# eloimoliner/BABE

Measured on AMD Instinct MI355X. Metric: audio-sec/s (blind BWE, 10 s @ 44.1 kHz clips, 35 EDM steps 2nd order), whole job, higher is better.
Workload: dtype f32

## Files before the change

### babe_amd/csrc/common.h

```cpp
#pragma once
#include <hip/hip_runtime.h>
#include <cstdio>
#include <cstring>
#include <cstdint>

#define BABE_OK 0
#define BABE_ERR_ARG -1
#define BABE_ERR_HIP -2
#define BABE_ERR_UNSUPPORTED -3

void babe_set_error(const char* fmt, ...);

#define BABE_CHECK_ARG(cond, ...)                      \
    do {                                               \
        if (!(cond)) {                                 \
            babe_set_error(__VA_ARGS__);               \
            return BABE_ERR_ARG;                       \
        }                                              \
    } while (0)

#define BABE_TRY(call)                                 \
    do {                                               \
        const int rc__ = (call);                       \
        if (rc__ != BABE_OK) return rc__;              \
    } while (0)

#define BABE_LAUNCH_CHECK()                                                       \
    do {                                                                          \
        hipError_t e__ = hipGetLastError();                                       \
        if (e__ != hipSuccess) {                                                  \
            babe_set_error("%s:%d HIP launch error: %s", __FILE__, __LINE__,      \
                           hipGetErrorString(e__));                               \
            return BABE_ERR_HIP;                                                  \
        }                                                                         \
    } while (0)

static inline int cdiv(long a, long b) { return (int)((a + b - 1) / b); }

#include <atomic>
#include <initializer_list>
static inline hipError_t babe_lds_optin(std::atomic<unsigned long long>& done, std::initializer_list<const void*> fns,
                                        int bytes) {
    int dev = 0;
    hipError_t e = hipGetDevice(&dev);
    if (e != hipSuccess) return e;
    const unsigned long long bit = 1ull << (dev & 63);
    if (done.load(std::memory_order_acquire) & bit) return hipSuccess;
    for (const void* f : fns) {
        e = hipFuncSetAttribute(f, hipFuncAttributeMaxDynamicSharedMemorySize, bytes);
        if (e != hipSuccess) return e;
    }
    done.fetch_or(bit, std::memory_order_release);
    return hipSuccess;
}

__device__ __forceinline__ long sgpr_pin(long v) {
    asm volatile("" : "+s"(v));
    return v;
}
struct ChanSrc {
    const float* p1;
    long d2, cs1, cs2;
    int split;
    __device__ __forceinline__ void init(const float* in, long bs, long cs, const float* in2, long bs2, long cs2_,
                                         int split_, int b) {
        p1 = in + (long)b * bs;
        d2 = sgpr_pin(in2 ? (long)((in2 + (long)b * bs2) - p1) : 0);
        cs1 = sgpr_pin(cs);
        cs2 = sgpr_pin(in2 ? cs2_ : cs);
        split = split_;
    }
    __device__ __forceinline__ const float* operator()(int ci) const {
        const bool first = ci < split;
        const long cs = first ? cs1 : cs2;
        const int c = first ? ci : ci - split;
        return p1 + ((first ? 0 : d2) + (long)c * cs);
    }
};

__device__ __forceinline__ double wave_sum(double v) {
#pragma unroll
    for (int o = 32; o > 0; o >>= 1) v += __shfl_xor(v, o, 64);
    return v;
}
__device__ __forceinline__ float wave_sumf(float v) {
#pragma unroll
    for (int o = 32; o > 0; o >>= 1) v += __shfl_xor(v, o, 64);
    return v;
}

template <int NW>
__device__ __forceinline__ double block_sum(double v, double* sh) {
    v = wave_sum(v);
    if ((threadIdx.x & 63) == 0) sh[threadIdx.x >> 6] = v;
    __syncthreads();
    double t = sh[0];
#pragma unroll
    for (int w = 1; w < NW; ++w) t += sh[w];
    return t;
}
```

### babe_amd/csrc/misc.hip

```cpp
#include "common.h"
#include "../../include/babe_hip.h"
#include "prof.h"
#include <cstdarg>
#include <vector>

static thread_local char g_err[512] = "";

void babe_set_error(const char* fmt, ...) {
    va_list ap;
    va_start(ap, fmt);
    vsnprintf(g_err, sizeof(g_err), fmt, ap);
    va_end(ap);
}
extern "C" const char* babe_last_error(void) { return g_err; }
extern "C" const char* babe_version(void) { return "babe_hip 0.1 (gfx950)"; }

namespace {
struct ProfRec { hipEvent_t e0, e1; int slot; void* stream; double flops; };
struct Prof {
    bool on = false;
    int conv_slot_override = -1;
    std::vector<ProfRec> rec;
    size_t used = 0;
    double bytes[BABE_NSLOTS] = {}, flops[BABE_NSLOTS] = {}, exec[BABE_NSLOTS] = {};
// ... 22 lines not shown
    r.stream = stream;
    r.flops = flops;
    (void)hipEventRecord(r.e0, (hipStream_t)stream);
    g_prof.bytes[slot] += bytes;
    g_prof.flops[slot] += flops;
    g_prof.exec[slot] += exec_flops;
    g_prof.open = true;
}
extern "C" void babe_prof_end(void* stream) {
    if (!g_prof.open) return;
    (void)hipEventRecord(g_prof.rec[g_prof.used++].e1, (hipStream_t)stream);
    g_prof.open = false;
}
extern "C" int babe_prof_nslots(void) { return BABE_NSLOTS; }
extern "C" const char* babe_prof_slot_name(int slot) { return (slot >= 0 && slot < BABE_NSLOTS) ? kSlotNames[slot] : ""; }
extern "C" int babe_prof_enable(int on) {
    if (on < 0) return g_prof.on ? 1 : 0;
    g_prof.on = on != 0;
    g_prof.open = false;
    return BABE_OK;
}
extern "C" int babe_prof_conv_slot(int slot) {
    g_prof.conv_slot_override = (slot >= 0 && slot < BABE_NSLOTS) ? slot : -1;
    return BABE_OK;
}
extern "C" int babe_prof_read(double* ms, double* bytes, double* flops, double* exec_flops, long* launches) {
    for (int i = 0; i < BABE_NSLOTS; ++i) {
        if (ms) ms[i] = 0;
        if (launches) launches[i] = 0;
    }
    for (size_t i = 0; i < g_prof.used; ++i) {
        ProfRec& r = g_prof.rec[i];
        if (hipEventSynchronize(r.e1) != hipSuccess) {
            babe_set_error("prof_read: hipEventSynchronize failed");
            return BABE_ERR_HIP;
        }
        float t = 0;
        (void)hipEventElapsedTime(&t, r.e0, r.e1);
        if (ms) ms[r.slot] += t;
        if (launches) launches[r.slot]++;
    }
    for (int i = 0; i < BABE_NSLOTS; ++i) {
        if (bytes) bytes[i] = g_prof.bytes[i];
        if (flops) flops[i] = g_prof.flops[i];
        if (exec_flops) exec_flops[i] = g_prof.exec[i];
        g_prof.bytes[i] = g_prof.flops[i] = g_prof.exec[i] = 0;
    }
    g_prof.used = 0;
    return BABE_OK;
}
extern "C" long babe_prof_timeline(double* t0_ms, double* t1_ms, int* slot, int* lane, double* flops, long cap) {
    std::vector<void*> streams;
    long n = 0;
    for (size_t i = 0; i < g_prof.used && n < cap; ++i, ++n) {
        ProfRec& r = g_prof.rec[i];
        if (hipEventSynchronize(r.e1) != hipSuccess) {
            babe_set_error("prof_timeline: hipEventSynchronize failed");
            return BABE_ERR_HIP;
        }
        float a = 0, b = 0;
        (void)hipEventElapsedTime(&a, g_prof.rec[0].e0, r.e0);
        (void)hipEventElapsedTime(&b, g_prof.rec[0].e0, r.e1);
        size_t k = 0;
        while (k < streams.size() && streams[k] != r.stream) ++k;
        if (k == streams.size()) streams.push_back(r.stream);
        if (t0_ms) t0_ms[n] = a;
        if (t1_ms) t1_ms[n] = b;
        if (slot) slot[n] = r.slot;
        if (lane) lane[n] = (int)k;
        if (flops) flops[n] = r.flops;
    }
    return n;
}
extern "C" long babe_prof_pending(void) { return (long)g_prof.used; }
extern "C" int babe_prof_dispatch_counts(long* counts, int reset) {
    for (int i = 0; i < BABE_NSLOTS; ++i) {
        if (counts) counts[i] = g_prof.dispatch[i];
        if (reset) g_prof.dispatch[i] = 0;
    }
    return BABE_OK;
}

namespace {
template <int V>
__global__ __launch_bounds__(256) void axpby4d_kernel(const float* __restrict__ in, long in_bs, long in_cs,
                                                      float* __restrict__ out, long out_bs, long out_cs, int C, long n,
                                                      float alpha, float beta) {
    const int b = blockIdx.y / C, c = blockIdx.y % C;
    const float* x = in + (long)b * in_bs + (long)c * in_cs;
    float* y = out + (long)b * out_bs + (long)c * out_cs;
    const long stride = (long)gridDim.x * blockDim.x * V;
    for (long i = ((long)blockIdx.x * blockDim.x + threadIdx.x) * V; i < n; i += stride) {
        if constexpr (V == 4) {
            typedef float f32x4 __attribute__((ext_vector_type(4)));
            f32x4 v = alpha * *reinterpret_cast<const f32x4*>(x + i);
            if (beta != 0.f) v += beta * *reinterpret_cast<const f32x4*>(y + i);
            *reinterpret_cast<f32x4*>(y + i) = v;
        } else {
            const float v = alpha * x[i];
            y[i] = (beta != 0.f) ? v + beta * y[i] : v;
        }
    }
}

__global__ __launch_bounds__(256) void axpby2_4d_kernel(const float* __restrict__ xin, long x_bs, long x_cs,
                                                        const float* __restrict__ yin, long y_bs, long y_cs,
                                                        float* __restrict__ out, long out_bs, long out_cs, int C, long n,
                                                        float alpha, float beta) {
    typedef float f32x4 __attribute__((ext_vector_type(4)));
    const int b = blockIdx.y / C, c = blockIdx.y % C;
    const float* x = xin + (long)b * x_bs + (long)c * x_cs;
    const float* y = yin + (long)b * y_bs + (long)c * y_cs;
    float* o = out + (long)b * out_bs + (long)c * out_cs;
    const long stride = (long)gridDim.x * blockDim.x * 4;
    for (long i = ((long)blockIdx.x * blockDim.x + threadIdx.x) * 4; i < n; i += stride) {
        const f32x4 xv = *reinterpret_cast<const f32x4*>(x + i), yv = *reinterpret_cast<const f32x4*>(y + i);
        f32x4 v;
#pragma unroll
        for (int e = 0; e < 4; ++e) {
#pragma clang fp contract(off)
            const float p = alpha * xv[e], q = beta * yv[e];
            v[e] = p + q;
        }
        *reinterpret_cast<f32x4*>(o + i) = v;
    }
}

__global__ __launch_bounds__(256) void fill4d_kernel(float* __restrict__ out, long out_bs, long out_cs, int C, long n, float value) {
    const int b = blockIdx.y / C, c = blockIdx.y % C;
    float* y = out + (long)b * out_bs + (long)c * out_cs;
    for (long i = (long)blockIdx.x * blockDim.x + threadIdx.x; i < n; i += (long)gridDim.x * blockDim.x) y[i] = value;
}

__global__ __launch_bounds__(256) void linear_kernel(const float* __restrict__ x, const float* __restrict__ W,
                                                     const float* __restrict__ bias, float* __restrict__ out, int B,
                                                     int K, int J, int relu) {
    const int j = blockIdx.x * 4 + (threadIdx.x >> 6);
    const int lane = threadIdx.x & 63;
    if (j >= J) return;
    for (int b = 0; b < B; ++b) {
        float s = 0.f;
        for (int k = lane; k < K; k += 64) s += x[(long)b * K + k] * W[(long)j * K + k];
        s = wave_sumf(s);
        if (lane == 0) {
            s += bias ? bias[j] : 0.f;
            if (relu) s = s > 0.f ? s : 0.f;
            out[(long)b * J + j] = s;
        }
    }
}

__global__ void rff_kernel(const float* __restrict__ cnoise, const float* __restrict__ freq, float* __restrict__ out,
                           int B, int R) {
    const int i = blockIdx.x * blockDim.x + threadIdx.x;
    if (i >= B * R) return;
    const int b = i / R, r = i % R;
    const float tab = (6.283185307179586f * cnoise[b]) * freq[r];
    out[(long)b * 2 * R + r] = sinf(tab);
    out[(long)b * 2 * R + R + r] = cosf(tab);
}
}

extern "C" int babe_axpby4d(const float* in, long in_bs, long in_cs, float* out, long out_bs, long out_cs, int B,
                            int C, int F, int T, float alpha, float beta, void* stream) {
    BABE_CHECK_ARG(in && out && B > 0 && C > 0 && F > 0 && T > 0, "axpby4d: bad arguments");
    BABE_CHECK_ARG((long)B * C <= 65535 && F <= 65535, "axpby4d: grid too large");
    const long n = (long)F * T;
    auto al16 = [](const void* p) { return ((uintptr_t)p & 15) == 0; };
    const bool v4 = (n % 4 == 0) && al16(in) && al16(out) && in_bs % 4 == 0 && in_cs % 4 == 0 && out_bs % 4 == 0 &&
                    out_cs % 4 == 0;
    BabeProfScope prof(BABE_SLOT_AXPBY, (beta != 0.f ? 12.0 : 8.0) * B * C * (double)n, 0, 0, stream);
    if (v4) {
        int bx = cdiv(n / 4, 256);
        if (bx > 64) bx = 64;
        hipLaunchKernelGGL(axpby4d_kernel<4>, dim3(bx, B * C), dim3(256), 0, (hipStream_t)stream, in, in_bs, in_cs, out,
                           out_bs, out_cs, C, n, alpha, beta);
    } else {
        int bx = cdiv(n, 256);
        if (bx > 64) bx = 64;
        hipLaunchKernelGGL(axpby4d_kernel<1>, dim3(bx, B * C), dim3(256), 0, (hipStream_t)stream, in, in_bs, in_cs, out,
                           out_bs, out_cs, C, n, alpha, beta);
    }
    BABE_LAUNCH_CHECK();
    return BABE_OK;
}

extern "C" int babe_axpby2_4d(const float* x, long x_bs, long x_cs, const float* y, long y_bs, long y_cs, float* out, long out_bs,
                              long out_cs, int B, int C, int F, int T, float alpha, float beta, void* stream) {
    BABE_CHECK_ARG(x && y && out && B > 0 && C > 0 && F > 0 && T > 0, "axpby2_4d: bad arguments");
    BABE_CHECK_ARG((long)B * C <= 65535, "axpby2_4d: grid too large");
    const long n = (long)F * T;
    auto al16 = [](const void* p) { return ((uintptr_t)p & 15) == 0; };
    BABE_CHECK_ARG(n % 4 == 0 && al16(x) && al16(y) && al16(out) && x_bs % 4 == 0 && x_cs % 4 == 0 && y_bs % 4 == 0 && y_cs % 4 == 0 &&
                       out_bs % 4 == 0 && out_cs % 4 == 0,
                   "axpby2_4d: planes must be 16-byte aligned with F*T %% 4 == 0 (use two babe_axpby4d calls otherwise)");
    BabeProfScope prof(BABE_SLOT_AXPBY, 12.0 * B * C * (double)n, 0, 0, stream);
    int bx = cdiv(n / 4, 256);
    if (bx > 64) bx = 64;
    hipLaunchKernelGGL(axpby2_4d_kernel, dim3(bx, B * C), dim3(256), 0, (hipStream_t)stream, x, x_bs, x_cs, y, y_bs, y_cs, out, out_bs,
                       out_cs, C, n, alpha, beta);
    BABE_LAUNCH_CHECK();
    return BABE_OK;
}

extern "C" int babe_fill4d(float* out, long out_bs, long out_cs, int B, int C, int F, int T, float value, void* stream) {
    BABE_CHECK_ARG(out && B > 0 && C > 0 && F > 0 && T > 0 && (long)B * C <= 65535, "fill4d: bad arguments");
    const long n = (long)F * T;
    int bx = cdiv(n, 1024);
    if (bx > 64) bx = 64;
    hipLaunchKernelGGL(fill4d_kernel, dim3(bx, B * C), dim3(256), 0, (hipStream_t)stream, out, out_bs, out_cs, C, n, value);
    BABE_LAUNCH_CHECK();
    return BABE_OK;
}

extern "C" int babe_linear(const float* x, const float* W, const float* bias, float* out, int B, int K, int J,
                           int relu, void* stream) {
    BABE_CHECK_ARG(x && W && out && B > 0 && K > 0 && J > 0, "linear: bad arguments");
    BabeProfScope prof(BABE_SLOT_FILM, 4.0 * ((double)J * K + (double)B * (K + J)), 2.0 * B * J * K, 0, stream);
    hipLaunchKernelGGL(linear_kernel, dim3(cdiv(J, 4)), dim3(256), 0, (hipStream_t)stream, x, W, bias, out, B, K, J,
                       relu);
    BABE_LAUNCH_CHECK();
    return BABE_OK;
}

extern "C" int babe_rff(const float* cnoise, const float* freq, float* out, int B, int R, void* stream) {
    BABE_CHECK_ARG(cnoise && freq && out && B > 0 && R > 0, "rff: bad arguments");
    BabeProfScope prof(BABE_SLOT_FILM, 4.0 * B * (1 + 3 * R), 0, 0, stream);
    hipLaunchKernelGGL(rff_kernel, dim3(cdiv(B * R, 64)), dim3(64), 0, (hipStream_t)stream, cnoise, freq, out, B, R);
    BABE_LAUNCH_CHECK();
    return BABE_OK;
}
```

### babe_amd/csrc/norm.hip

```cpp
#include "common.h"
#include "../../include/babe_hip.h"
#include "prof.h"
#include "gelu.h"
#include <cstdlib>

namespace {

using babe_gelu::gelu_f;
using babe_gelu::gelu_grad_f;

template <int NV>
__device__ __forceinline__ void block_reduce(double (&v)[NV], double* sh) {
#pragma unroll
    for (int k = 0; k < NV; ++k) v[k] = wave_sum(v[k]);
    const int lane = threadIdx.x & 63, wave = threadIdx.x >> 6;
    if (lane == 0) {
#pragma unroll
        for (int k = 0; k < NV; ++k) sh[wave * NV + k] = v[k];
    }
    __syncthreads();
    if (threadIdx.x == 0) {
#pragma unroll
        for (int k = 0; k < NV; ++k) v[k] = 0;
        for (int w = 0; w < (int)(blockDim.x >> 6); ++w) {
#pragma unroll
            for (int k = 0; k < NV; ++k) v[k] += sh[w * NV + k];
        }
    }
}

struct GnStat {
    float mean, sd, r;
};
__device__ __forceinline__ GnStat gn_stat(double s0, double s1, long n, float eps) {
    const double mean = s0 / (double)n;
    double var = (s1 - (double)n * mean * mean) / (double)(n - 1);
    if (var < 0) var = 0;
    const float sd = (float)sqrt(var);
    return {(float)mean, sd, 1.f / (sd + eps)};
}
__device__ __forceinline__ void gn_stat_store(float* __restrict__ stats, int bg, const GnStat st) {
    stats[bg * 3 + 0] = st.mean;
    stats[bg * 3 + 1] = st.sd;
    stats[bg * 3 + 2] = st.r;
}

__device__ __forceinline__ void half_wave_sum2(double& s0, double& s1) {
#pragma unroll
    for (int o = 16; o >= 1; o >>= 1) {
        s0 += __shfl_xor(s0, o, 32);
        s1 += __shfl_xor(s1, o, 32);
    }
}
template <typename P>
__device__ __forceinline__ void gn_part_sum32(P part, long row, int S, int sub, double& s0, double& s1) {
    s0 = 0, s1 = 0;
    for (int q = sub; q < S; q += 32) {
        s0 += part[(row + q) * 2];
        s1 += part[(row + q) * 2 + 1];
    }
    half_wave_sum2(s0, s1);
}

template <bool FUSED>
__global__ __launch_bounds__(256) void gn_partial_kernel(const float* __restrict__ x, double* __restrict__ part,
                                                         long n, int S, int* __restrict__ ticket,
                                                         const float* __restrict__ gamma, const float* __restrict__ film,
                                                         long film_bs, float* __restrict__ stats, float* __restrict__ scale,
                                                         int C, int G, float eps) {
    __shared__ double sh[8];
    __shared__ int last_sh;
    __shared__ float r_sh;
    const int s = blockIdx.x;
    const long bg = blockIdx.y;
    const long chunk = ((n / 4 + S - 1) / S) * 4;
    const long beg = (long)s * chunk;
    long end = beg + chunk;
    if (end > n) end = n;
    const float* p = x + bg * n;
    double s0 = 0, s1 = 0;
    if (beg < end) {
        const long nv = (end - beg) / 4;
        const float4* p4 = reinterpret_cast<const float4*>(p + beg);
        long i = threadIdx.x;
        for (; i + 3 * (long)blockDim.x < nv; i += 4 * (long)blockDim.x) {
            const float4 v0 = p4[i], v1 = p4[i + blockDim.x], v2 = p4[i + 2 * blockDim.x], v3 = p4[i + 3 * blockDim.x];
            s0 += ((double)v0.x + (double)v0.y + (double)v0.z + (double)v0.w) + ((double)v1.x + (double)v1.y + (double)v1.z + (double)v1.w) +
                  ((double)v2.x + (double)v2.y + (double)v2.z + (double)v2.w) + ((double)v3.x + (double)v3.y + (double)v3.z + (double)v3.w);
            s1 += ((double)v0.x * v0.x + (double)v0.y * v0.y + (double)v0.z * v0.z + (double)v0.w * v0.w) +
                  ((double)v1.x * v1.x + (double)v1.y * v1.y + (double)v1.z * v1.z + (double)v1.w * v1.w) +
                  ((double)v2.x * v2.x + (double)v2.y * v2.y + (double)v2.z * v2.z + (double)v2.w * v2.w) +
                  ((double)v3.x * v3.x + (double)v3.y * v3.y + (double)v3.z * v3.z + (double)v3.w * v3.w);
        }
        for (; i < nv; i += blockDim.x) {
            const float4 v = p4[i];
            s0 += (double)v.x + (double)v.y + (double)v.z + (double)v.w;
            s1 += (double)v.x * v.x + (double)v.y * v.y + (double)v.z * v.z + (double)v.w * v.w;
        }
        for (long i = beg + nv * 4 + threadIdx.x; i < end; i += blockDim.x) {
            const double v = p[i];
            s0 += v;
            s1 += v * v;
        }
    }
    double sum[2] = {s0, s1};
    block_reduce(sum, sh);
    if (threadIdx.x == 0) {
        part[(bg * S + s) * 2] = sum[0];
        part[(bg * S + s) * 2 + 1] = sum[1];
    }
    if constexpr (FUSED) {
        if (threadIdx.x == 0) {
            __threadfence();
            const int old = atomicAdd(&ticket[bg], 1);
            last_sh = old == S - 1;
            if (old == S - 1) ticket[bg] = 0;
        }
        __syncthreads();
        if (!last_sh) return;
        __threadfence();
        const int b = (int)(bg / G), g = (int)(bg % G);
        if (threadIdx.x < 32) {
            const volatile double* vp = part;
            double t0, t1;
            gn_part_sum32(vp, bg * S, S, threadIdx.x, t0, t1);
            if (threadIdx.x == 0) {
                const GnStat st = gn_stat(t0, t1, n, eps);
                gn_stat_store(stats, b * G + g, st);
                r_sh = st.r;
            }
        }
        __syncthreads();
        const int cg = C / G;
        for (int j = threadIdx.x; j < cg; j += blockDim.x) {
            const int c = g * cg + j;
            scale[b * C + c] = gamma[c] * (film[(long)b * film_bs + c] + 1.f) * r_sh;
        }
    }
}

__global__ void gn_finalize_kernel(const double* __restrict__ part, const float* __restrict__ gamma,
                                   const float* __restrict__ film, long film_bs, float* __restrict__ stats,
                                   float* __restrict__ scale, int C, int G, long n, int S, float eps) {
    const int b = blockIdx.x;
    __shared__ float rstd_sh[64];
    const int sub = threadIdx.x & 31;
    for (int g = threadIdx.x >> 5; g < G; g += blockDim.x >> 5) {
        double s0, s1;
        gn_part_sum32(part, (long)(b * G + g) * S, S, sub, s0, s1);
        if (sub != 0) continue;
        const GnStat st = gn_stat(s0, s1, n, eps);
        gn_stat_store(stats, b * G + g, st);
        rstd_sh[g] = st.r;
    }
    __syncthreads();
    const int cg = C / G;
    for (int c = threadIdx.x; c < C; c += blockDim.x)
        scale[b * C + c] = gamma[c] * (film[(long)b * film_bs + c] + 1.f) * rstd_sh[c / cg];
}

__global__ __launch_bounds__(256) void scale_gelu_kernel(const float* __restrict__ x, const float* __restrict__ scale,
                                                         float* __restrict__ a, int C, long hw) {
    const int c = blockIdx.y, b = blockIdx.z;
    const float sc = scale[b * C + c];
    const long base = ((long)b * C + c) * hw;
    const long nv = hw / 4;
    const float4* x4 = reinterpret_cast<const float4*>(x + base);
    float4* a4 = reinterpret_cast<float4*>(a + base);
    for (long i = (long)blockIdx.x * blockDim.x + threadIdx.x; i < nv; i += (long)gridDim.x * blockDim.x) {
        float4 v = x4[i];
        v.x = gelu_f(v.x * sc);
        v.y = gelu_f(v.y * sc);
        v.z = gelu_f(v.z * sc);
        v.w = gelu_f(v.w * sc);
        a4[i] = v;
    }
    if (blockIdx.x == 0)
        for (long i = nv * 4 + threadIdx.x; i < hw; i += blockDim.x) a[base + i] = gelu_f(x[base + i] * sc);
}

__global__ __launch_bounds__(256) void scale_gelu_fin_kernel(const float* __restrict__ x, const double* __restrict__ part,
                                                             const float* __restrict__ gamma, const float* __restrict__ film,
                                                             long film_bs, float* __restrict__ stats, float* __restrict__ scale,
                                                             float* __restrict__ a, int C, int G, long hw, long n, int S,
                                                             float eps) {
    __shared__ float sc_sh;
    __shared__ double red_sh[512];
    const int c = blockIdx.y, b = blockIdx.z;
    const int cg = C / G, g = c / cg;
    {
        double t0 = 0, t1 = 0;
        for (int q = threadIdx.x; q < S; q += 256) {
            t0 += part[((long)(b * G + g) * S + q) * 2];
            t1 += part[((long)(b * G + g) * S + q) * 2 + 1];
        }
        red_sh[threadIdx.x * 2] = t0;
        red_sh[threadIdx.x * 2 + 1] = t1;
    }
    __syncthreads();
    if (threadIdx.x < 32) {
        double t0 = 0, t1 = 0;
#pragma unroll
        for (int j = 0; j < 8; ++j) {
            t0 += red_sh[(threadIdx.x + 32 * j) * 2];
            t1 += red_sh[(threadIdx.x + 32 * j) * 2 + 1];
        }
        half_wave_sum2(t0, t1);
        if (threadIdx.x == 0) {
            const GnStat st = gn_stat(t0, t1, n, eps);
            const float scv = gamma[c] * (film[(long)b * film_bs + c] + 1.f) * st.r;
            sc_sh = scv;
            if (blockIdx.x == 0) {
                scale[b * C + c] = scv;
                if (c == g * cg) gn_stat_store(stats, b * G + g, st);
            }
        }
    }
    __syncthreads();
    const float sc = sc_sh;
    const long base = ((long)b * C + c) * hw;
    const long nv = hw / 4;
    const float4* x4 = reinterpret_cast<const float4*>(x + base);
    float4* a4 = reinterpret_cast<float4*>(a + base);
    for (long i = (long)blockIdx.x * blockDim.x + threadIdx.x; i < nv; i += (long)gridDim.x * blockDim.x) {
        float4 v = x4[i];
        v.x = gelu_f(v.x * sc);
        v.y = gelu_f(v.y * sc);
        v.z = gelu_f(v.z * sc);
        v.w = gelu_f(v.w * sc);
        a4[i] = v;
    }
    if (blockIdx.x == 0)
        for (long i = nv * 4 + threadIdx.x; i < hw; i += blockDim.x) a[base + i] = gelu_f(x[base + i] * sc);
}

typedef __bf16 bf16x8_n __attribute__((ext_vector_type(8)));
__global__ __launch_bounds__(256) void scale_gelu_units_kernel(const float* __restrict__ x, const float* __restrict__ scale,
                                                               bf16x8_n* __restrict__ au, int C, int F, int T) {
    const int g = blockIdx.y, b = blockIdx.z;
    const int Q = T >> 2, PI = Q + 1;
    const long hw = (long)F * T;
    float sc[8];
#pragma unroll
    for (int j = 0; j < 8; ++j) sc[j] = scale[b * C + 8 * g + j];
    const float* xb = x + ((long)b * C + 8 * g) * hw;
    bf16x8_n* ab = au + ((long)b * (C >> 3) + g) * F * 4 * PI;
    const long nq = (long)F * Q;
    for (long i = (long)blockIdx.x * blockDim.x + threadIdx.x; i < nq; i += (long)gridDim.x * blockDim.x) {
        const int f = (int)(i / Q), q = (int)(i - (long)f * Q);
        float4 v[8];
#pragma unroll
        for (int j = 0; j < 8; ++j) v[j] = *reinterpret_cast<const float4*>(xb + j * hw + (long)f * T + 4 * q);
        bf16x8_n u0, u1, u2, u3, z;
#pragma unroll
        for (int j = 0; j < 8; ++j) {
            u0[j] = (__bf16)gelu_f(v[j].x * sc[j]);
            u1[j] = (__bf16)gelu_f(v[j].y * sc[j]);
            u2[j] = (__bf16)gelu_f(v[j].z * sc[j]);
            u3[j] = (__bf16)gelu_f(v[j].w * sc[j]);
            z[j] = (__bf16)0.f;
        }
        bf16x8_n* row = ab + (long)f * 4 * PI;
        row[1 * PI + q] = u0;
        row[2 * PI + q] = u1;
        row[3 * PI + q] = u2;
        row[q + 1] = u3;
        if (q == 0) row[0] = z;
        if (q == Q - 1) {
            row[1 * PI + Q] = z;
            row[2 * PI + Q] = z;
            row[3 * PI + Q] = z;
        }
    }
}

template <bool GELU>
__global__ __launch_bounds__(256) void gn_bwd_partial_kernel(const float* __restrict__ x, const float* __restrict__ dadu,
                                                             const float* __restrict__ scale,
                                                             double* __restrict__ part, int C, int G, long hw, int S) {
    __shared__ double sh[4];
    const int s = blockIdx.x;
    const int bg = blockIdx.y;
    const int b = bg / G, g = bg % G;
    const int cg = C / G;
    const long n = (long)cg * hw;
    const long chunk = ((n / 4 + S - 1) / S) * 4;
    const long beg = (long)s * chunk;
    long end = beg + chunk;
    if (end > n) end = n;
    const long base = ((long)b * C + (long)g * cg) * hw;
    double s0 = 0;
    if (beg < end) {
        const int c_lo = (int)(beg / hw), c_hi = (int)((end - 1) / hw);
        for (int cl = c_lo; cl <= c_hi; ++cl) {
            const long lo = beg > (long)cl * hw ? beg : (long)cl * hw;
            const long hi = end < (long)(cl + 1) * hw ? end : (long)(cl + 1) * hw;
            const float sc = scale[b * C + g * cg + cl];
            double sc_sum = 0;
            auto term = [&](const float4 xv, float4 dv) {
                if (GELU) {
                    dv.x *= gelu_grad_f(xv.x * sc);
                    dv.y *= gelu_grad_f(xv.y * sc);
                    dv.z *= gelu_grad_f(xv.z * sc);
                    dv.w *= gelu_grad_f(xv.w * sc);
                }
                return (double)dv.x * xv.x + (double)dv.y * xv.y + (double)dv.z * xv.z + (double)dv.w * xv.w;
            };
            const long st = (long)blockDim.x * 4;
            long i = lo + (long)threadIdx.x * 4;
            for (; i + st < hi; i += 2 * st) {
                const float4 x0 = *reinterpret_cast<const float4*>(x + base + i);
                const float4 d0 = *reinterpret_cast<const float4*>(dadu + base + i);
                const float4 x1 = *reinterpret_cast<const float4*>(x + base + i + st);
                const float4 d1 = *reinterpret_cast<const float4*>(dadu + base + i + st);
                sc_sum += term(x0, d0);
                sc_sum += term(x1, d1);
            }
            for (; i < hi; i += st)
                sc_sum += term(*reinterpret_cast<const float4*>(x + base + i), *reinterpret_cast<const float4*>(dadu + base + i));
            s0 += (double)sc * sc_sum;
        }
    }
    double sum[1] = {s0};
    block_reduce(sum, sh);
    if (threadIdx.x == 0) part[(long)bg * S + s] = sum[0];
}

template <bool GELU>
__global__ __launch_bounds__(256) void gn_bwd_apply_kernel(const float* __restrict__ x, const float* __restrict__ da,
                                                           const float* __restrict__ gy,
                                                           const float* __restrict__ scale,
                                                           const float* __restrict__ stats,
                                                           const double* __restrict__ part, float* __restrict__ gx,
                                                           float rbeta, int C, int G, long hw, int S, float eps,
                                                           const float* __restrict__ acc, float ca, float cb) {
    const int c = blockIdx.y, b = blockIdx.z;
    const int cg = C / G;
    const int g = c / cg;
    const long n = (long)cg * hw;
    __shared__ double S1_sh;
    if (threadIdx.x < 64) {
        double v = 0;
        for (int s = threadIdx.x; s < S; s += 64) v += part[(long)(b * G + g) * S + s];
        v = wave_sum(v);
        if (threadIdx.x == 0) S1_sh = v;
    }
    __syncthreads();
    const double S1 = S1_sh;
    const float mean = stats[(b * G + g) * 3 + 0];
    const float sd = stats[(b * G + g) * 3 + 1];
    const double se = (double)sd + eps;
    const float coef = (sd > 0.f) ? (float)(S1 * se / ((double)(n - 1) * sd * se * se)) : 0.f;
    const float sc = scale[b * C + c];
    const long base = ((long)b * C + c) * hw;
    const long nv = hw / 4;
    const float4* x4 = reinterpret_cast<const float4*>(x + base);
    const float4* d4 = reinterpret_cast<const float4*>(da + base);
    const float4* g4 = gy ? reinterpret_cast<const float4*>(gy + base) : nullptr;
    float4* o4 = reinterpret_cast<float4*>(gx + base);
    for (long i = (long)blockIdx.x * blockDim.x + threadIdx.x; i < nv; i += (long)gridDim.x * blockDim.x) {
        const float4 xv = x4[i];
        float4 dv = d4[i];
        if (GELU) {
            dv.x *= gelu_grad_f(xv.x * sc);
            dv.y *= gelu_grad_f(xv.y * sc);
            dv.z *= gelu_grad_f(xv.z * sc);
            dv.w *= gelu_grad_f(xv.w * sc);
        }
        float4 o;
        o.x = sc * dv.x - (xv.x - mean) * coef;
        o.y = sc * dv.y - (xv.y - mean) * coef;
        o.z = sc * dv.z - (xv.z - mean) * coef;
        o.w = sc * dv.w - (xv.w - mean) * coef;
        if (g4) {
            const float4 gv = g4[i];
            o.x += rbeta * gv.x;
            o.y += rbeta * gv.y;
            o.z += rbeta * gv.z;
            o.w += rbeta * gv.w;
        }
        if (acc) {
#pragma clang fp contract(off)
            const float4 av = reinterpret_cast<const float4*>(acc + base)[i];
            const float px = ca * av.x, py = ca * av.y, pz = ca * av.z, pw = ca * av.w;
            const float qx = cb * o.x, qy = cb * o.y, qz = cb * o.z, qw = cb * o.w;
            o.x = px + qx;
            o.y = py + qy;
            o.z = pz + qz;
            o.w = pw + qw;
        }
        o4[i] = o;
    }
}

int plane_blocks(long hw) {
    const int bx = cdiv(hw / 4, 256 * 4);
    return bx < 1 ? 1 : bx > 64 ? 64 : bx;
}

}

extern "C" long babe_gn_splits(long n) {
    const long s = n / 16384;
    return s < 1 ? 1 : s > 64 ? 64 : s;
}

extern "C" int babe_gn_partial(const float* x, double* part, int B, int G, long n, int S, void* stream) {
    BABE_CHECK_ARG(x && part && B > 0 && G > 0 && n > 1 && S > 0, "gn_partial: bad arguments");
    BABE_CHECK_ARG(n % 4 == 0, "gn_partial: group size %ld not a multiple of 4", n);
    BabeProfScope prof(BABE_SLOT_GN_STATS, 4.0 * B * G * (double)n, 0, 0, stream);
    hipLaunchKernelGGL(gn_partial_kernel<false>, dim3(S, B * G), dim3(256), 0, (hipStream_t)stream, x, part, n, S,
                       (int*)nullptr, (const float*)nullptr, (const float*)nullptr, 0L, (float*)nullptr, (float*)nullptr, 0, 1, 0.f);
    BABE_LAUNCH_CHECK();
    return BABE_OK;
}

extern "C" int babe_gn_stats(const float* x, double* part, int* ticket, const float* gamma, const float* film, long film_bs,
                             float* stats, float* scale, int B, int C, int G, long n, int S, float eps, void* stream) {
    BABE_CHECK_ARG(x && part && ticket && gamma && film && stats && scale && B > 0 && G > 0 && n > 1 && S > 0, "gn_stats: bad arguments");
    BABE_CHECK_ARG(n % 4 == 0 && G <= 64 && C % G == 0, "gn_stats: n=%ld C=%d G=%d unsupported", n, C, G);
    BabeProfScope prof(BABE_SLOT_GN_STATS, 4.0 * B * G * (double)n, 0, 0, stream);
    hipLaunchKernelGGL(gn_partial_kernel<true>, dim3(S, B * G), dim3(256), 0, (hipStream_t)stream, x, part, n, S, ticket, gamma,
                       film, film_bs, stats, scale, C, G, eps);
    BABE_LAUNCH_CHECK();
    return BABE_OK;
}

extern "C" int babe_gn_finalize(const double* part, const float* gamma, const float* film, long film_bs, float* stats,
                                float* scale, int B, int C, int G, long n, int S, float eps, void* stream) {
    BABE_CHECK_ARG(part && gamma && film && stats && scale, "gn_finalize: null pointer");
    BABE_CHECK_ARG(G <= 64 && C % G == 0, "gn_finalize: C=%d G=%d unsupported", C, G);
    BabeProfScope prof(BABE_SLOT_GN_STATS, 0, 0, 0, stream);
    hipLaunchKernelGGL(gn_finalize_kernel, dim3(B), dim3(256), 0, (hipStream_t)stream, part, gamma, film, film_bs,
                       stats, scale, C, G, n, S, eps);
    BABE_LAUNCH_CHECK();
    return BABE_OK;
}

extern "C" int babe_scale_gelu(const float* x, const float* scale, float* a, int B, int C, long hw, void* stream) {
    BABE_CHECK_ARG(x && scale && a && B > 0 && C > 0 && hw > 0, "scale_gelu: bad arguments");
    BABE_CHECK_ARG(hw % 4 == 0, "scale_gelu: plane size %ld not a multiple of 4", hw);
    BabeProfScope prof(BABE_SLOT_SCALE_GELU, 8.0 * B * C * (double)hw, 0, 0, stream);
    const int bx = plane_blocks(hw);
    hipLaunchKernelGGL(scale_gelu_kernel, dim3(bx, C, B), dim3(256), 0, (hipStream_t)stream, x, scale, a, C, hw);
    BABE_LAUNCH_CHECK();
    return BABE_OK;
}

extern "C" int babe_scale_gelu_fin(const float* x, const double* part, const float* gamma, const float* film, long film_bs,
                                   float* stats, float* scale, float* a, int B, int C, int G, long hw, int S, float eps,
                                   void* stream) {
    BABE_CHECK_ARG(x && part && gamma && film && stats && scale && a && B > 0 && C > 0 && hw > 0 && S > 0, "scale_gelu_fin: bad arguments");
    BABE_CHECK_ARG(hw % 4 == 0 && G <= 64 && C % G == 0, "scale_gelu_fin: hw=%ld C=%d G=%d unsupported", hw, C, G);
    BabeProfScope prof(BABE_SLOT_SCALE_GELU, 8.0 * B * C * (double)hw, 0, 0, stream);
    const int bx = plane_blocks(hw);
    const long n = (long)(C / G) * hw;
    hipLaunchKernelGGL(scale_gelu_fin_kernel, dim3(bx, C, B), dim3(256), 0, (hipStream_t)stream, x, part, gamma, film, film_bs,
                       stats, scale, a, C, G, hw, n, S, eps);
    BABE_LAUNCH_CHECK();
    return BABE_OK;
}

extern "C" long babe_units_size(int C, int F, int T) { return (long)(C / 8) * F * 4 * (T / 4 + 1); }

extern "C" int babe_scale_gelu_units(const float* x, const float* scale, void* au, int B, int C, int F, int T,
                                     void* stream) {
    BABE_CHECK_ARG(x && scale && au && B > 0 && C > 0 && F > 0 && T > 0, "scale_gelu_units: bad arguments");
    BABE_CHECK_ARG(T % 4 == 0 && C % 8 == 0, "scale_gelu_units: T=%d C=%d unsupported (need T %% 4 == 0, C %% 8 == 0)", T, C);
    BABE_CHECK_ARG(((uintptr_t)x & 15) == 0 && ((uintptr_t)au & 15) == 0, "scale_gelu_units: unaligned pointer");
    BabeProfScope prof(BABE_SLOT_SCALE_GELU, 6.0 * B * C * (double)F * T, 0, 0, stream);
    int bx = cdiv((long)F * (T / 4), 256 * 2);
    if (bx < 1) bx = 1;
    if (bx > 256) bx = 256;
    hipLaunchKernelGGL(scale_gelu_units_kernel, dim3(bx, C / 8, B), dim3(256), 0, (hipStream_t)stream, x, scale,
                       (bf16x8_n*)au, C, F, T);
    BABE_LAUNCH_CHECK();
    return BABE_OK;
}

static int gn_bwd_partial_launch(bool gelu, const float* x, const float* da, const float* scale, double* part, int B, int C, int G,
                                 long hw, int S, void* stream) {
    BABE_CHECK_ARG(x && da && scale && part, "gn_bwd_partial: null pointer");
    BABE_CHECK_ARG(hw % 4 == 0 && C % G == 0, "gn_bwd_partial: hw=%ld C=%d G=%d unsupported", hw, C, G);
    BabeProfScope prof(BABE_SLOT_GN_BWD_PARTIAL, 8.0 * B * C * (double)hw, 0, 0, stream);
    if (gelu)
        hipLaunchKernelGGL(gn_bwd_partial_kernel<true>, dim3(S, B * G), dim3(256), 0, (hipStream_t)stream, x, da, scale, part, C, G,
                           hw, S);
    else
        hipLaunchKernelGGL(gn_bwd_partial_kernel<false>, dim3(S, B * G), dim3(256), 0, (hipStream_t)stream, x, da, scale, part, C, G,
                           hw, S);
    BABE_LAUNCH_CHECK();
    return BABE_OK;
}

extern "C" int babe_gn_bwd_partial(const float* x, const float* da, const float* scale, double* part, int B, int C,
                                   int G, long hw, int S, void* stream) {
    return gn_bwd_partial_launch(true, x, da, scale, part, B, C, G, hw, S, stream);
}

extern "C" int babe_gn_bwd_partial_nogelu(const float* x, const float* da, const float* scale, double* part, int B, int C,
                                          int G, long hw, int S, void* stream) {
    return gn_bwd_partial_launch(false, x, da, scale, part, B, C, G, hw, S, stream);
}

static int gn_bwd_apply_launch(bool gelu, const float* acc, float ca, float cb, const float* x, const float* da, const float* gy, const float* scale,
                                 const float* stats, const double* part, float* gx, float rbeta, int B, int C, int G,
                                 long hw, int S, float eps, void* stream) {
    BABE_CHECK_ARG(x && da && scale && stats && part && gx, "gn_bwd_apply: null pointer");
    BABE_CHECK_ARG(hw % 4 == 0 && C % G == 0, "gn_bwd_apply: hw=%ld C=%d G=%d unsupported", hw, C, G);
    BabeProfScope prof(BABE_SLOT_GN_BWD_APPLY, ((gy ? 16.0 : 12.0) + (acc ? 4.0 : 0.0)) * B * C * (double)hw, 0, 0, stream);
    const int bx = plane_blocks(hw);
    if (gelu)
        hipLaunchKernelGGL(gn_bwd_apply_kernel<true>, dim3(bx, C, B), dim3(256), 0, (hipStream_t)stream, x, da, gy, scale, stats,
                           part, gx, rbeta, C, G, hw, S, eps, acc, ca, cb);
    else
        hipLaunchKernelGGL(gn_bwd_apply_kernel<false>, dim3(bx, C, B), dim3(256), 0, (hipStream_t)stream, x, da, gy, scale, stats,
                           part, gx, rbeta, C, G, hw, S, eps, acc, ca, cb);
    BABE_LAUNCH_CHECK();
    return BABE_OK;
}

extern "C" int babe_gn_bwd_apply(const float* x, const float* da, const float* gy, const float* scale,
                                 const float* stats, const double* part, float* gx, float rbeta, int B, int C, int G,
                                 long hw, int S, float eps, void* stream) {
    return gn_bwd_apply_launch(true, nullptr, 0.f, 0.f, x, da, gy, scale, stats, part, gx, rbeta, B, C, G, hw, S, eps, stream);
}

extern "C" int babe_gn_bwd_apply_nogelu(const float* x, const float* da, const float* gy, const float* scale,
                                        const float* stats, const double* part, float* gx, float rbeta, int B, int C, int G,
                                        long hw, int S, float eps, void* stream) {
    return gn_bwd_apply_launch(false, nullptr, 0.f, 0.f, x, da, gy, scale, stats, part, gx, rbeta, B, C, G, hw, S, eps, stream);
}

extern "C" int babe_gn_bwd_apply_merge(const float* x, const float* da, const float* gy, const float* scale,
                                 const float* stats, const double* part, float* gx, float rbeta, int B, int C, int G,
                                 long hw, int S, float eps, void* stream, const float* acc, float ca, float cb) {
    BABE_CHECK_ARG(acc && ((uintptr_t)acc & 15) == 0, "gn_bwd_apply_merge: acc must be a 16-byte aligned dense tensor");
    return gn_bwd_apply_launch(true, acc, ca, cb, x, da, gy, scale, stats, part, gx, rbeta, B, C, G, hw, S, eps, stream);
}
```

Before: 2.595.

## Software-pipeline elementwise and groupnorm kernels with double-buffered prefetch loads

```diff
diff --git a/babe_amd/csrc/common.h b/babe_amd/csrc/common.h
--- a/babe_amd/csrc/common.h
+++ b/babe_amd/csrc/common.h
@@ -89,6 +89,37 @@
     return v;
 }
 
+__device__ __forceinline__ void pipeline_head() {
+    asm volatile("" ::: "memory");
+    __builtin_amdgcn_sched_barrier(0);
+}
+
+__device__ __forceinline__ float4 ld16(const float* base, int i) {
+    return *reinterpret_cast<const float4*>(reinterpret_cast<const char*>(base) + (unsigned)i * 16u);
+}
+__device__ __forceinline__ void st16(float* base, int i, const float4 v) {
+    *reinterpret_cast<float4*>(reinterpret_cast<char*>(base) + (unsigned)i * 16u) = v;
+}
+
+template <typename T, typename Load, typename Use>
+__device__ __forceinline__ void sweep2(T a, T b, int i, const int st, const int nv, Load load, Use use) {
+    for (; i + 3 * st < nv; i += 2 * st) {
+        use(a, i);
+        a = load(i + 2 * st);
+        pipeline_head();
+        use(b, i + st);
+        b = load(i + 3 * st);
+        pipeline_head();
+    }
+    if (i < nv) {
+        use(a, i);
+        const bool third = i + 2 * st < nv;
+        if (third) a = load(i + 2 * st);
+        if (i + st < nv) use(b, i + st);
+        if (third) use(a, i + 2 * st);
+    }
+}
+
 template <int NW>
 __device__ __forceinline__ double block_sum(double v, double* sh) {
     v = wave_sum(v);
diff --git a/babe_amd/csrc/misc.hip b/babe_amd/csrc/misc.hip
--- a/babe_amd/csrc/misc.hip
+++ b/babe_amd/csrc/misc.hip
@@ -128,24 +128,53 @@
 }
 
 namespace {
-template <int V>
+typedef float f32x4 __attribute__((ext_vector_type(4)));
+__device__ __forceinline__ f32x4 ld16v(const float* base, int i) {
+    return *reinterpret_cast<const f32x4*>(reinterpret_cast<const char*>(base) + (unsigned)i * 16u);
+}
+__device__ __forceinline__ void st16v(float* base, int i, const f32x4 v) {
+    *reinterpret_cast<f32x4*>(reinterpret_cast<char*>(base) + (unsigned)i * 16u) = v;
+}
+
+template <bool BETA>
+__device__ __forceinline__ float axpby_one(float alpha, float x, float beta, float y) {
+    float p;
+    {
+#pragma clang fp contract(off)
+        p = alpha * x;
+    }
+    return BETA ? __builtin_fmaf(beta, y, p) : p;
+}
+
+template <int V, bool BETA>
 __global__ __launch_bounds__(256) void axpby4d_kernel(const float* __restrict__ in, long in_bs, long in_cs,
                                                       float* __restrict__ out, long out_bs, long out_cs, int C, long n,
                                                       float alpha, float beta) {
     const int b = blockIdx.y / C, c = blockIdx.y % C;
     const float* x = in + (long)b * in_bs + (long)c * in_cs;
     float* y = out + (long)b * out_bs + (long)c * out_cs;
-    const long stride = (long)gridDim.x * blockDim.x * V;
-    for (long i = ((long)blockIdx.x * blockDim.x + threadIdx.x) * V; i < n; i += stride) {
-        if constexpr (V == 4) {
-            typedef float f32x4 __attribute__((ext_vector_type(4)));
-            f32x4 v = alpha * *reinterpret_cast<const f32x4*>(x + i);
-            if (beta != 0.f) v += beta * *reinterpret_cast<const f32x4*>(y + i);
-            *reinterpret_cast<f32x4*>(y + i) = v;
-        } else {
-            const float v = alpha * x[i];
-            y[i] = (beta != 0.f) ? v + beta * y[i] : v;
-        }
+    if constexpr (V == 4) {
+        struct In {
+            f32x4 x, y;
+        };
+        const int nv = (int)(n / 4), i0 = blockIdx.x * blockDim.x + threadIdx.x, st = gridDim.x * blockDim.x;
+        auto load = [&](int i) {
+            In v;
+            v.x = ld16v(x, i);
+            if constexpr (BETA) v.y = ld16v(y, i);
+            return v;
+        };
+        const In in0 = load(i0 < nv ? i0 : nv - 1), in1 = load(i0 + st < nv ? i0 + st : nv - 1);
+        sweep2(in0, in1, i0, st, nv, load, [&](const In& in, int i) {
+            f32x4 v;
+#pragma unroll
+            for (int e = 0; e < 4; ++e) v[e] = axpby_one<BETA>(alpha, in.x[e], beta, BETA ? in.y[e] : 0.f);
+            st16v(y, i, v);
+        });
+    } else {
+        const long stride = (long)gridDim.x * blockDim.x;
+        for (long i = (long)blockIdx.x * blockDim.x + threadIdx.x; i < n; i += stride)
+            y[i] = axpby_one<BETA>(alpha, x[i], beta, BETA ? y[i] : 0.f);
     }
 }
 
@@ -153,23 +182,26 @@
                                                         const float* __restrict__ yin, long y_bs, long y_cs,
                                                         float* __restrict__ out, long out_bs, long out_cs, int C, long n,
                                                         float alpha, float beta) {
-    typedef float f32x4 __attribute__((ext_vector_type(4)));
     const int b = blockIdx.y / C, c = blockIdx.y % C;
     const float* x = xin + (long)b * x_bs + (long)c * x_cs;
     const float* y = yin + (long)b * y_bs + (long)c * y_cs;
     float* o = out + (long)b * out_bs + (long)c * out_cs;
-    const long stride = (long)gridDim.x * blockDim.x * 4;
-    for (long i = ((long)blockIdx.x * blockDim.x + threadIdx.x) * 4; i < n; i += stride) {
-        const f32x4 xv = *reinterpret_cast<const f32x4*>(x + i), yv = *reinterpret_cast<const f32x4*>(y + i);
+    struct In {
+        f32x4 x, y;
+    };
+    const int nv = (int)(n / 4), i0 = blockIdx.x * blockDim.x + threadIdx.x, st = gridDim.x * blockDim.x;
+    auto load = [&](int i) { return In{ld16v(x, i), ld16v(y, i)}; };
+    const In in0 = load(i0 < nv ? i0 : nv - 1), in1 = load(i0 + st < nv ? i0 + st : nv - 1);
+    sweep2(in0, in1, i0, st, nv, load, [&](const In& in, int i) {
         f32x4 v;
 #pragma unroll
         for (int e = 0; e < 4; ++e) {
 #pragma clang fp contract(off)
-            const float p = alpha * xv[e], q = beta * yv[e];
+            const float p = alpha * in.x[e], q = beta * in.y[e];
             v[e] = p + q;
         }
-        *reinterpret_cast<f32x4*>(o + i) = v;
-    }
+        st16v(o, i, v);
+    });
 }
 
 __global__ __launch_bounds__(256) void fill4d_kernel(float* __restrict__ out, long out_bs, long out_cs, int C, long n, float value) {
@@ -212,6 +244,7 @@
     BABE_CHECK_ARG(in && out && B > 0 && C > 0 && F > 0 && T > 0, "axpby4d: bad arguments");
     BABE_CHECK_ARG((long)B * C <= 65535 && F <= 65535, "axpby4d: grid too large");
     const long n = (long)F * T;
+    BABE_CHECK_ARG(n < (1L << 30), "axpby4d: plane of %ld elements too large", n);
     auto al16 = [](const void* p) { return ((uintptr_t)p & 15) == 0; };
     const bool v4 = (n % 4 == 0) && al16(in) && al16(out) && in_bs % 4 == 0 && in_cs % 4 == 0 && out_bs % 4 == 0 &&
                     out_cs % 4 == 0;
@@ -219,13 +252,13 @@
     if (v4) {
         int bx = cdiv(n / 4, 256);
         if (bx > 64) bx = 64;
-        hipLaunchKernelGGL(axpby4d_kernel<4>, dim3(bx, B * C), dim3(256), 0, (hipStream_t)stream, in, in_bs, in_cs, out,
-                           out_bs, out_cs, C, n, alpha, beta);
+        hipLaunchKernelGGL((beta != 0.f ? axpby4d_kernel<4, true> : axpby4d_kernel<4, false>), dim3(bx, B * C), dim3(256), 0,
+                           (hipStream_t)stream, in, in_bs, in_cs, out, out_bs, out_cs, C, n, alpha, beta);
     } else {
         int bx = cdiv(n, 256);
         if (bx > 64) bx = 64;
-        hipLaunchKernelGGL(axpby4d_kernel<1>, dim3(bx, B * C), dim3(256), 0, (hipStream_t)stream, in, in_bs, in_cs, out,
-                           out_bs, out_cs, C, n, alpha, beta);
+        hipLaunchKernelGGL((beta != 0.f ? axpby4d_kernel<1, true> : axpby4d_kernel<1, false>), dim3(bx, B * C), dim3(256), 0,
+                           (hipStream_t)stream, in, in_bs, in_cs, out, out_bs, out_cs, C, n, alpha, beta);
     }
     BABE_LAUNCH_CHECK();
     return BABE_OK;
@@ -236,6 +269,7 @@
     BABE_CHECK_ARG(x && y && out && B > 0 && C > 0 && F > 0 && T > 0, "axpby2_4d: bad arguments");
     BABE_CHECK_ARG((long)B * C <= 65535, "axpby2_4d: grid too large");
     const long n = (long)F * T;
+    BABE_CHECK_ARG(n < (1L << 30), "axpby2_4d: plane of %ld elements too large", n);
     auto al16 = [](const void* p) { return ((uintptr_t)p & 15) == 0; };
     BABE_CHECK_ARG(n % 4 == 0 && al16(x) && al16(y) && al16(out) && x_bs % 4 == 0 && x_cs % 4 == 0 && y_bs % 4 == 0 && y_cs % 4 == 0 &&
                        out_bs % 4 == 0 && out_cs % 4 == 0,
diff --git a/babe_amd/csrc/norm.hip b/babe_amd/csrc/norm.hip
--- a/babe_amd/csrc/norm.hip
+++ b/babe_amd/csrc/norm.hip
@@ -26,6 +26,30 @@
 #pragma unroll
             for (int k = 0; k < NV; ++k) v[k] += sh[w * NV + k];
         }
+    }
+}
+
+template <typename T, typename Load, typename Use>
+__device__ __forceinline__ void pipelined_rounds(int rounds, Load load, Use use) {
+    if (rounds <= 0) return;
+    T a = load(0), b;
+    pipeline_head();
+    int k = 1;
+    for (; k + 1 < rounds; k += 2) {
+        b = load(k);
+        pipeline_head();
+        use(a);
+        a = load(k + 1);
+        pipeline_head();
+        use(b);
+    }
+    if (k < rounds) {
+        b = load(k);
+        pipeline_head();
+        use(a);
+        use(b);
+    } else {
+        use(a);
     }
 }
 
@@ -162,21 +186,23 @@
 __global__ __launch_bounds__(256) void scale_gelu_kernel(const float* __restrict__ x, const float* __restrict__ scale,
                                                          float* __restrict__ a, int C, long hw) {
     const int c = blockIdx.y, b = blockIdx.z;
+    const long base = ((long)b * C + c) * hw;
+    const int nv = (int)(hw / 4);
+    const float* xp = x + base;
+    float* ap = a + base;
+    const int i0 = blockIdx.x * blockDim.x + threadIdx.x, st = gridDim.x * blockDim.x;
+    auto load = [&](int i) { return ld16(xp, i); };
+    const float4 v0 = load(i0 < nv ? i0 : nv - 1), v1 = load(i0 + st < nv ? i0 + st : nv - 1);
     const float sc = scale[b * C + c];
-    const long base = ((long)b * C + c) * hw;
-    const long nv = hw / 4;
-    const float4* x4 = reinterpret_cast<const float4*>(x + base);
-    float4* a4 = reinterpret_cast<float4*>(a + base);
-    for (long i = (long)blockIdx.x * blockDim.x + threadIdx.x; i < nv; i += (long)gridDim.x * blockDim.x) {
-        float4 v = x4[i];
+    sweep2(v0, v1, i0, st, nv, load, [&](float4 v, int i) {
         v.x = gelu_f(v.x * sc);
         v.y = gelu_f(v.y * sc);
         v.z = gelu_f(v.z * sc);
         v.w = gelu_f(v.w * sc);
-        a4[i] = v;
-    }
+        st16(ap, i, v);
+    });
     if (blockIdx.x == 0)
-        for (long i = nv * 4 + threadIdx.x; i < hw; i += blockDim.x) a[base + i] = gelu_f(x[base + i] * sc);
+        for (long i = (long)nv * 4 + threadIdx.x; i < hw; i += blockDim.x) a[base + i] = gelu_f(x[base + i] * sc);
 }
 
 __global__ __launch_bounds__(256) void scale_gelu_fin_kernel(const float* __restrict__ x, const double* __restrict__ part,
@@ -188,15 +214,45 @@
     __shared__ double red_sh[512];
     const int c = blockIdx.y, b = blockIdx.z;
     const int cg = C / G, g = c / cg;
-    {
-        double t0 = 0, t1 = 0;
-        for (int q = threadIdx.x; q < S; q += 256) {
-            t0 += part[((long)(b * G + g) * S + q) * 2];
-            t1 += part[((long)(b * G + g) * S + q) * 2 + 1];
-        }
-        red_sh[threadIdx.x * 2] = t0;
-        red_sh[threadIdx.x * 2 + 1] = t1;
-    }
+    const long base = ((long)b * C + c) * hw;
+    const int nv = (int)(hw / 4);
+    const float* xp = x + base;
+    float* ap = a + base;
+    const int i0 = blockIdx.x * blockDim.x + threadIdx.x, st = gridDim.x * blockDim.x;
+    auto load = [&](int i) { return ld16(xp, i); };
+    constexpr int SLOTS = 4;
+    const double* prow = part + (long)(b * G + g) * S * 2;
+    double t0 = 0, t1 = 0;
+    double p0[SLOTS], p1[SLOTS];
+#pragma unroll
+    for (int k = 0; k < SLOTS; ++k) {
+        const int q = threadIdx.x + 256 * k, qc = q < S ? q : S - 1;
+        p0[k] = prow[(long)qc * 2];
+        p1[k] = prow[(long)qc * 2 + 1];
+    }
+    const float4 v0 = load(i0 < nv ? i0 : nv - 1), v1 = load(i0 + st < nv ? i0 + st : nv - 1);
+#pragma unroll
+    for (int k = 0; k < SLOTS; ++k)
+        if ((int)threadIdx.x + 256 * k < S) {
+            t0 += p0[k];
+            t1 += p1[k];
+        }
+    for (int qb = threadIdx.x + 256 * SLOTS; qb < S; qb += 256 * SLOTS) {
+#pragma unroll
+        for (int k = 0; k < SLOTS; ++k) {
+            const int q = qb + 256 * k, qc = q < S ? q : S - 1;
+            p0[k] = prow[(long)qc * 2];
+            p1[k] = prow[(long)qc * 2 + 1];
+        }
+#pragma unroll
+        for (int k = 0; k < SLOTS; ++k)
+            if (qb + 256 * k < S) {
+                t0 += p0[k];
+                t1 += p1[k];
+            }
+    }
+    red_sh[threadIdx.x * 2] = t0;
+    red_sh[threadIdx.x * 2 + 1] = t1;
     __syncthreads();
     if (threadIdx.x < 32) {
         double t0 = 0, t1 = 0;
@@ -218,20 +274,15 @@
     }
     __syncthreads();
     const float sc = sc_sh;
-    const long base = ((long)b * C + c) * hw;
-    const long nv = hw / 4;
-    const float4* x4 = reinterpret_cast<const float4*>(x + base);
-    float4* a4 = reinterpret_cast<float4*>(a + base);
-    for (long i = (long)blockIdx.x * blockDim.x + threadIdx.x; i < nv; i += (long)gridDim.x * blockDim.x) {
-        float4 v = x4[i];
+    sweep2(v0, v1, i0, st, nv, load, [&](float4 v, int i) {
         v.x = gelu_f(v.x * sc);
         v.y = gelu_f(v.y * sc);
         v.z = gelu_f(v.z * sc);
         v.w = gelu_f(v.w * sc);
-        a4[i] = v;
-    }
+        st16(ap, i, v);
+    });
     if (blockIdx.x == 0)
-        for (long i = nv * 4 + threadIdx.x; i < hw; i += blockDim.x) a[base + i] = gelu_f(x[base + i] * sc);
+        for (long i = (long)nv * 4 + threadIdx.x; i < hw; i += blockDim.x) a[base + i] = gelu_f(x[base + i] * sc);
 }
 
 typedef __bf16 bf16x8_n __attribute__((ext_vector_type(8)));
@@ -275,7 +326,7 @@
 }
 
 template <bool GELU>
-__global__ __launch_bounds__(256) void gn_bwd_partial_kernel(const float* __restrict__ x, const float* __restrict__ dadu,
+__global__ __launch_bounds__(256, 8) void gn_bwd_partial_kernel(const float* __restrict__ x, const float* __restrict__ dadu,
                                                              const float* __restrict__ scale,
                                                              double* __restrict__ part, int C, int G, long hw, int S) {
     __shared__ double sh[4];
@@ -306,18 +357,26 @@
                 }
                 return (double)dv.x * xv.x + (double)dv.y * xv.y + (double)dv.z * xv.z + (double)dv.w * xv.w;
             };
-            const long st = (long)blockDim.x * 4;
-            long i = lo + (long)threadIdx.x * 4;
-            for (; i + st < hi; i += 2 * st) {
-                const float4 x0 = *reinterpret_cast<const float4*>(x + base + i);
-                const float4 d0 = *reinterpret_cast<const float4*>(dadu + base + i);
-                const float4 x1 = *reinterpret_cast<const float4*>(x + base + i + st);
-                const float4 d1 = *reinterpret_cast<const float4*>(dadu + base + i + st);
-                sc_sum += term(x0, d0);
-                sc_sum += term(x1, d1);
+            const float* xs = x + base + lo;
+            const float* ds = dadu + base + lo;
+            const int nv = (int)((hi - lo) / 4), st = blockDim.x;
+            int i = threadIdx.x;
+            struct X2 {
+                float4 x0, d0, x1, d1;
+            };
+            auto load2 = [&](int j) { return X2{ld16(xs, j), ld16(ds, j), ld16(xs, j + st), ld16(ds, j + st)}; };
+            auto add2 = [&](const X2& v) {
+                sc_sum += term(v.x0, v.d0);
+                sc_sum += term(v.x1, v.d1);
+            };
+            const int rounds = nv / (2 * st);
+            pipelined_rounds<X2>(rounds, [&](int k) { return load2(i + k * 2 * st); }, add2);
+            i += rounds * 2 * st;
+            if (i + st < nv) {
+                add2(load2(i));
+                i += 2 * st;
             }
-            for (; i < hi; i += st)
-                sc_sum += term(*reinterpret_cast<const float4*>(x + base + i), *reinterpret_cast<const float4*>(dadu + base + i));
+            for (; i < nv; i += st) sc_sum += term(ld16(xs, i), ld16(ds, i));
             s0 += (double)sc * sc_sum;
         }
     }
@@ -326,8 +385,11 @@
     if (threadIdx.x == 0) part[(long)bg * S + s] = sum[0];
 }
 
-template <bool GELU>
-__global__ __launch_bounds__(256) void gn_bwd_apply_kernel(const float* __restrict__ x, const float* __restrict__ da,
+struct GnApplyIn {
+    float4 x, d, g, a;
+};
+template <bool GELU, bool GY, bool ACC>
+__global__ __launch_bounds__(256, 8) void gn_bwd_apply_kernel(const float* __restrict__ x, const float* __restrict__ da,
                                                            const float* __restrict__ gy,
                                                            const float* __restrict__ scale,
                                                            const float* __restrict__ stats,
@@ -338,29 +400,38 @@
     const int cg = C / G;
     const int g = c / cg;
     const long n = (long)cg * hw;
-    __shared__ double S1_sh;
-    if (threadIdx.x < 64) {
-        double v = 0;
-        for (int s = threadIdx.x; s < S; s += 64) v += part[(long)(b * G + g) * S + s];
-        v = wave_sum(v);
-        if (threadIdx.x == 0) S1_sh = v;
-    }
-    __syncthreads();
-    const double S1 = S1_sh;
+    const long base = ((long)b * C + c) * hw;
+    const int nv = (int)(hw / 4);
+    const float* xp = x + base;
+    const float* dp = da + base;
+    const float* gp = GY ? gy + base : nullptr;
+    const float* ap = ACC ? acc + base : nullptr;
+    float* op = gx + base;
+    const int i0 = blockIdx.x * blockDim.x + threadIdx.x, st = gridDim.x * blockDim.x;
+    auto load = [&](int i) {
+        GnApplyIn v;
+        v.x = ld16(xp, i);
+        v.d = ld16(dp, i);
+        if constexpr (GY) v.g = ld16(gp, i);
+        if constexpr (ACC) v.a = ld16(ap, i);
+        return v;
+    };
+    const int lane = threadIdx.x & 63;
+    const double pv = part[(long)(b * G + g) * S + (lane < S ? lane : S - 1)];
+    const GnApplyIn in0 = load(i0 < nv ? i0 : nv - 1), in1 = load(i0 + st < nv ? i0 + st : nv - 1);
+    pipeline_head();
+    double S1 = 0;
+    if (lane < S) S1 += pv;
+    for (int s = lane + 64; s < S; s += 64) S1 += part[(long)(b * G + g) * S + s];
+    S1 = wave_sum(S1);
     const float mean = stats[(b * G + g) * 3 + 0];
     const float sd = stats[(b * G + g) * 3 + 1];
     const double se = (double)sd + eps;
     const float coef = (sd > 0.f) ? (float)(S1 * se / ((double)(n - 1) * sd * se * se)) : 0.f;
     const float sc = scale[b * C + c];
-    const long base = ((long)b * C + c) * hw;
-    const long nv = hw / 4;
-    const float4* x4 = reinterpret_cast<const float4*>(x + base);
-    const float4* d4 = reinterpret_cast<const float4*>(da + base);
-    const float4* g4 = gy ? reinterpret_cast<const float4*>(gy + base) : nullptr;
-    float4* o4 = reinterpret_cast<float4*>(gx + base);
-    for (long i = (long)blockIdx.x * blockDim.x + threadIdx.x; i < nv; i += (long)gridDim.x * blockDim.x) {
-        const float4 xv = x4[i];
-        float4 dv = d4[i];
+    sweep2(in0, in1, i0, st, nv, load, [&](const GnApplyIn& in, int i) {
+        const float4 xv = in.x;
+        float4 dv = in.d;
         if (GELU) {
             dv.x *= gelu_grad_f(xv.x * sc);
             dv.y *= gelu_grad_f(xv.y * sc);
@@ -372,16 +443,16 @@
         o.y = sc * dv.y - (xv.y - mean) * coef;
         o.z = sc * dv.z - (xv.z - mean) * coef;
         o.w = sc * dv.w - (xv.w - mean) * coef;
-        if (g4) {
-            const float4 gv = g4[i];
+        if constexpr (GY) {
+            const float4 gv = in.g;
             o.x += rbeta * gv.x;
             o.y += rbeta * gv.y;
             o.z += rbeta * gv.z;
             o.w += rbeta * gv.w;
         }
-        if (acc) {
+        if constexpr (ACC) {
 #pragma clang fp contract(off)
-            const float4 av = reinterpret_cast<const float4*>(acc + base)[i];
+            const float4 av = in.a;
             const float px = ca * av.x, py = ca * av.y, pz = ca * av.z, pw = ca * av.w;
             const float qx = cb * o.x, qy = cb * o.y, qz = cb * o.z, qw = cb * o.w;
             o.x = px + qx;
@@ -389,8 +460,8 @@
             o.z = pz + qz;
             o.w = pw + qw;
         }
-        o4[i] = o;
-    }
+        st16(op, i, o);
+    });
 }
 
 int plane_blocks(long hw) {
@@ -440,6 +511,7 @@
 extern "C" int babe_scale_gelu(const float* x, const float* scale, float* a, int B, int C, long hw, void* stream) {
     BABE_CHECK_ARG(x && scale && a && B > 0 && C > 0 && hw > 0, "scale_gelu: bad arguments");
     BABE_CHECK_ARG(hw % 4 == 0, "scale_gelu: plane size %ld not a multiple of 4", hw);
+    BABE_CHECK_ARG(hw < (1L << 30), "scale_gelu: plane of %ld elements too large", hw);
     BabeProfScope prof(BABE_SLOT_SCALE_GELU, 8.0 * B * C * (double)hw, 0, 0, stream);
     const int bx = plane_blocks(hw);
     hipLaunchKernelGGL(scale_gelu_kernel, dim3(bx, C, B), dim3(256), 0, (hipStream_t)stream, x, scale, a, C, hw);
@@ -452,6 +524,7 @@
                                    void* stream) {
     BABE_CHECK_ARG(x && part && gamma && film && stats && scale && a && B > 0 && C > 0 && hw > 0 && S > 0, "scale_gelu_fin: bad arguments");
     BABE_CHECK_ARG(hw % 4 == 0 && G <= 64 && C % G == 0, "scale_gelu_fin: hw=%ld C=%d G=%d unsupported", hw, C, G);
+    BABE_CHECK_ARG(hw < (1L << 30), "scale_gelu_fin: plane of %ld elements too large", hw);
     BabeProfScope prof(BABE_SLOT_SCALE_GELU, 8.0 * B * C * (double)hw, 0, 0, stream);
     const int bx = plane_blocks(hw);
     const long n = (long)(C / G) * hw;
@@ -482,6 +555,7 @@
                                  long hw, int S, void* stream) {
     BABE_CHECK_ARG(x && da && scale && part, "gn_bwd_partial: null pointer");
     BABE_CHECK_ARG(hw % 4 == 0 && C % G == 0, "gn_bwd_partial: hw=%ld C=%d G=%d unsupported", hw, C, G);
+    BABE_CHECK_ARG(S > 0 && ((long)(C / G) * hw / 4 + S - 1) / S < (1L << 28), "gn_bwd_partial: hw=%ld in S=%d splits: split too large", hw, S);
     BabeProfScope prof(BABE_SLOT_GN_BWD_PARTIAL, 8.0 * B * C * (double)hw, 0, 0, stream);
     if (gelu)
         hipLaunchKernelGGL(gn_bwd_partial_kernel<true>, dim3(S, B * G), dim3(256), 0, (hipStream_t)stream, x, da, scale, part, C, G,
@@ -508,14 +582,18 @@
                                  long hw, int S, float eps, void* stream) {
     BABE_CHECK_ARG(x && da && scale && stats && part && gx, "gn_bwd_apply: null pointer");
     BABE_CHECK_ARG(hw % 4 == 0 && C % G == 0, "gn_bwd_apply: hw=%ld C=%d G=%d unsupported", hw, C, G);
+    BABE_CHECK_ARG(hw < (1L << 30) && S > 0, "gn_bwd_apply: hw=%ld S=%d unsupported", hw, S);
     BabeProfScope prof(BABE_SLOT_GN_BWD_APPLY, ((gy ? 16.0 : 12.0) + (acc ? 4.0 : 0.0)) * B * C * (double)hw, 0, 0, stream);
     const int bx = plane_blocks(hw);
-    if (gelu)
-        hipLaunchKernelGGL(gn_bwd_apply_kernel<true>, dim3(bx, C, B), dim3(256), 0, (hipStream_t)stream, x, da, gy, scale, stats,
-                           part, gx, rbeta, C, G, hw, S, eps, acc, ca, cb);
-    else
-        hipLaunchKernelGGL(gn_bwd_apply_kernel<false>, dim3(bx, C, B), dim3(256), 0, (hipStream_t)stream, x, da, gy, scale, stats,
-                           part, gx, rbeta, C, G, hw, S, eps, acc, ca, cb);
+    using Kern = void (*)(const float*, const float*, const float*, const float*, const float*, const double*, float*, float, int,
+                          int, long, int, float, const float*, float, float);
+    static const Kern kerns[8] = {
+        gn_bwd_apply_kernel<false, false, false>, gn_bwd_apply_kernel<false, false, true>,
+        gn_bwd_apply_kernel<false, true, false>,  gn_bwd_apply_kernel<false, true, true>,
+        gn_bwd_apply_kernel<true, false, false>,  gn_bwd_apply_kernel<true, false, true>,
+        gn_bwd_apply_kernel<true, true, false>,   gn_bwd_apply_kernel<true, true, true>};
+    hipLaunchKernelGGL(kerns[(gelu ? 4 : 0) + (gy ? 2 : 0) + (acc ? 1 : 0)], dim3(bx, C, B), dim3(256), 0, (hipStream_t)stream, x,
+                       da, gy, scale, stats, part, gx, rbeta, C, G, hw, S, eps, acc, ca, cb);
     BABE_LAUNCH_CHECK();
     return BABE_OK;
 }
```

Result: no change. 2.608, median of 6 (+0.5%).
